# Z1HaoC/YOLO-Dual

Measured on AMD Instinct MI355X. Metric: images/sec at 640x640 bs=16/GPU, higher is better.
Workload: dtype bf16; 1 GPU; YOLOv5-backbone (C3+SPPF) + UNet-lite SegmentHead, fwd+bwd+SGD/EMA step, 640x640, bs=16/GPU, CE+0.5*Dice, 12 classes (BASELINE configs[1]); global_batch=16, parallelism=dp1

## Files before the change

### yolo_dual_amd/csrc/igemm.hip

```cpp
#include "common.h"
#include <type_traits>
#include <stdlib.h>

#ifndef YDL_PF
#define YDL_PF 1
#endif
#define ROWB 144
#define GROWB 128
#define MAXTAPS 64

struct IgemmArgs {
    const void* A;
    const void* B;
    void* C;
    float* stats;
    int N, Hi, Wi, lda;
    int Kc;
    int Ho, Wo, ldc;
    int Cout;
    int Cst;
    int Hg, Wg;
    int in_mul, out_mul, out_h0, out_w0;
    int ntaps, Ttot;
    int accumulate;
// ... 1504 lines not shown
        browoff[i] = co < p.Cout ? (unsigned)co * p.ldb_bytes + (unsigned)((qs ^ ((row >> 1) & 7)) << 4) : 0xF0000000u;
    }
    const int spt = p.Kc >> 6;
    const int nsteps = 9 * spt;
    u32x4 rsA, rsB;
    {
        const unsigned long long pa = (unsigned long long)p.A, pb = (unsigned long long)p.B;
        rsA = u32x4{(unsigned)pa, (unsigned)(pa >> 32) & 0xffffu, p.bytesA, 0x00020000u};
        rsB = u32x4{(unsigned)pb, (unsigned)(pb >> 32) & 0xffffu, p.bytesB, 0x00020000u};
    }
    const unsigned lds0 = (unsigned)(size_t)(__attribute__((address_space(3))) unsigned char*)smem;
    const unsigned wave_lds = lds0 + (unsigned)wave * (8 * GROWB);
    auto issue_patch = [&](int cb) {
        const unsigned base = wave_lds + (unsigned)(ONEP ? 0 : (cb & 1)) * PBYTES;
        const unsigned kb = (unsigned)cb << 7;
#pragma unroll
        for (int i = 0; i < PP; ++i) {
            if (RPP * i + wave * 8 < HS_PROWS)
                lds_dma16(rsA, base + i * RPP * GROWB, poff[i] == 0xFFFFFFFFu ? 0xFFFFFFFFu : poff[i] + kb);
        }
    };
    auto issue_w = [&](int stg, int cbw, int woff) {
        const unsigned add = cbw < spt ? (unsigned)woff + ((unsigned)cbw << 7) : 0xF0000000u;
        const unsigned base = wave_lds + (unsigned)NPB * PBYTES + (unsigned)stg * RBYTES;
#pragma unroll
        for (int i = 0; i < BR; ++i) lds_dma16(rsB, base + i * RPP * GROWB, browoff[i] + add);
    };
    f32x4 acc[CT][PT];
#pragma unroll
    for (int c = 0; c < CT; ++c)
#pragma unroll
        for (int j = 0; j < PT; ++j) acc[c][j] = f32x4{0.f, 0.f, 0.f, 0.f};
    const int lrow = lane & 15, lgrp = lane >> 4;
    const int sw_w = (lrow >> 1) & 7;
    const unsigned char* const fa = ring + (wc * BNW + lrow) * GROWB;
    issue_patch(0);
    issue_w(0, 0, sTw[0]);
    int cb = 0, tap = 0;
    int dcur = sTd[0], wnx = sTw[1];
    for (int g = 0; g < nsteps; ++g) {
        asm volatile("s_waitcnt lgkmcnt(0)" ::: "memory");
        wait_vm_barrier<0>();
        const int t1 = tap == 8 ? 0 : tap + 1, c1 = tap == 8 ? cb + 1 : cb;
        const int t2 = t1 == 8 ? 0 : t1 + 1;
        const int dnx = sTd[t1], wnn = sTw[t2];
        issue_w((g + 1) & 1, c1, wnx);
        if constexpr (ONEP) {
            if (tap == 0 && cb > 0) {
                issue_patch(cb);
                wait_vm_barrier<0>();
            }
        } else {
            if (tap == 0 && cb + 1 < spt) issue_patch(cb + 1);
        }
        const unsigned char* const wst = fa + (g & 1) * RBYTES;
        const unsigned char* const pst = smem + (ONEP ? 0 : (cb & 1)) * PBYTES;
        int prow[PT];
#pragma unroll
        for (int j = 0; j < PT; ++j) prow[j] = (wp * PT + j + 1) * H_PW + (lrow + 1) + dcur;
#pragma unroll
        for (int half = 0; half < 2; ++half) {
            uint4 af[CT], bfr[PT];
            const int kq = lgrp + 4 * half;
#pragma unroll
            for (int c = 0; c < CT; ++c) af[c] = *(const uint4*)(wst + c * 16 * GROWB + ((kq ^ sw_w) << 4));
#pragma unroll
            for (int j = 0; j < PT; ++j) bfr[j] = *(const uint4*)(pst + prow[j] * GROWB + ((kq ^ ((prow[j] >> 1) & 7)) << 4));
#pragma unroll
            for (int c = 0; c < CT; ++c)
#pragma unroll
                for (int j = 0; j < PT; ++j) Mma<T>::run(af[c], bfr[j], acc[c][j]);
        }
        dcur = dnx; wnx = wnn; tap = t1; cb = c1;
    }
    asm volatile("s_waitcnt lgkmcnt(0)" ::: "memory");
    wait_vm_barrier<0>();
    igemm2_epilogue<BM, BN, NW, WP>(p, acc, smem, 0, n0, mtile, BM, 16, 8, n * p.Ho + h0, w0);
}

__device__ __forceinline__ void buf_store16_asm(const u32x4& v, unsigned off, const u32x4& rsrc) {
    asm volatile("buffer_store_dwordx4 %0, %1, %2, 0 offen\n\ts_nop 1" ::"v"(v), "v"(off), "s"(rsrc) : "memory");
}
#define WR_PW 34
typedef __attribute__((ext_vector_type(16))) float f32x16_t;
template <int CO, bool STATS, int NW>
__global__ __launch_bounds__(NW * 64, 2) void igemm2w_kernel(const IgemmArgs p, int nblocks) {
    using T = bf16_t;
    constexpr int CG = CO / 32, PG = NW / CG, RW = 2, R = PG * RW;
    constexpr int NT = NW * 64, PR = NW * 8;
    constexpr int PROWS = (R + 2) * WR_PW;
    constexpr int PASSES = (PROWS + PR - 1) / PR;
    constexpr int PBYTES = PASSES * PR * GROWB;
    constexpr int BPX = R * 32;
    constexpr int NCH = CO / 8;
    constexpr int ORB = CO * 2;
    static_assert(BPX * NCH == 4 * NT && NT % NCH == 0, "four 16-byte store slots per thread, a fixed channel chunk per thread");
    extern __shared__ __attribute__((aligned(16))) unsigned char smem[];
    unsigned char* const stage = smem + 2 * PBYTES;
    float* const sred = (float*)smem;
    const int t = threadIdx.x, lane = t & 63;
    const int wave = __builtin_amdgcn_readfirstlane(t >> 6);
    const int cg = wave % CG, pg = wave / CG;
    const int ln = lane & 31, lh = lane >> 5;
    const int blocks_w = p.Wo >> 5, blocks_img = (p.Ho / R) * blocks_w;
    u32x4 rsA, rsC;
    {
        const unsigned long long pa = (unsigned long long)p.A, pc = (unsigned long long)p.C;
        rsA = u32x4{(unsigned)pa, (unsigned)(pa >> 32) & 0xffffu, p.bytesA, 0x00020000u};
        rsC = u32x4{(unsigned)pc, (unsigned)(pc >> 32) & 0xffffu, p.bytesC, 0x00020000u};
    }
    const unsigned lds0 = (unsigned)(size_t)(__attribute__((address_space(3))) unsigned char*)smem;
    const unsigned wave_lds = lds0 + (unsigned)wave * 1024u;
    const int rq = t >> 3, qs = t & 7;
    int pprc[PASSES];
#pragma unroll
    for (int i = 0; i < PASSES; ++i) {
        const int rho = i * PR + rq;
        pprc[i] = rho < PROWS ? ((rho / WR_PW) << 8) | (rho - (rho / WR_PW) * WR_PW) : (4000000 << 8);
    }
    auto block_origin = [&](int b, int& n, int& h0, int& w0) {
        n = b / blocks_img;
        const int rem = b - n * blocks_img;
        h0 = (rem / blocks_w) * R;
        w0 = (rem % blocks_w) << 5;
    };
    auto issue_patch = [&](int b, int buf) {
        int n, h0, w0;
        block_origin(b, n, h0, w0);
        const bool live = b < nblocks;
#pragma unroll
        for (int i = 0; i < PASSES; ++i) {
            const int rho = i * PR + rq;
            const int h = h0 - 1 + (pprc[i] >> 8), w = w0 - 1 + (pprc[i] & 255);
            const bool ok = live && (unsigned)h < (unsigned)p.Hi && (unsigned)w < (unsigned)p.Wi;
            const unsigned off = (unsigned)(((n * p.Hi + h) * p.Wi + w) * p.lda) * 2u + (unsigned)((qs ^ ((rho >> 1) & 7)) << 4);
            lds_dma16(rsA, wave_lds + (unsigned)buf * PBYTES + (unsigned)(i * PR * GROWB), ok ? off : 0xFFFFFFFFu);
        }
    };
    const int per = (nblocks + (int)gridDim.x - 1) / (int)gridDim.x;
    const int b0 = blockIdx.x * per, b1 = min(nblocks, b0 + per);
    issue_patch(b0, 0);
    uint4 wreg[9][4];
    {
        const __amdgpu_buffer_rsrc_t rsB = __builtin_amdgcn_make_buffer_rsrc((void*)p.B, 0, p.bytesB, 0x00020000);
        const int co = cg * 32 + ln;
#pragma unroll
        for (int tp = 0; tp < 9; ++tp)
#pragma unroll
            for (int ks = 0; ks < 4; ++ks) {
                const unsigned off = co < p.Cout ? (unsigned)co * p.ldb_bytes + (unsigned)(((int)p.wt[tp] * p.Kc + ks * 16 + lh * 8) * 2) : 0xFFFFFFFFu;
                const u32x4 v = __builtin_amdgcn_raw_buffer_load_b128(rsB, off, 0, 0);
                wreg[tp][ks] = make_uint4(v.x, v.y, v.z, v.w);
            }
    }
    int tapd[9];
#pragma unroll
    for (int tp = 0; tp < 9; ++tp) tapd[tp] = (int)p.dh[tp] * WR_PW + (int)p.dw[tp];
    float s1[STATS ? 8 : 1], s2[STATS ? 8 : 1];
#pragma unroll
    for (int e = 0; e < (STATS ? 8 : 1); ++e) { s1[e] = 0.f; s2[e] = 0.f; }
    const bool want_stats = STATS && p.stats != nullptr;
    int ridx_base = (pg * RW + 1) * WR_PW + ln + 1;
    asm volatile("s_waitcnt vmcnt(0)\n\ts_barrier" ::: "memory");
    int buf = 0;
    for (int b = b0; b < b1; ++b, buf ^= 1) {
        issue_patch(b + 1 < b1 ? b + 1 : nblocks, buf ^ 1);
        const unsigned char* const pst = smem + buf * PBYTES;
        f32x16_t acc[RW];
#pragma unroll
        for (int rb = 0; rb < RW; ++rb)
#pragma unroll
            for (int e = 0; e < 16; ++e) acc[rb][e] = 0.f;
        asm volatile("" : "+v"(ridx_base));
        uint4 fq[2][4];
        auto rd = [&](int tp, int rb, uint4 (&f)[4]) {
            const int ridx = ridx_base + rb * WR_PW + tapd[tp];
            const unsigned char* const rowp = pst + ridx * GROWB;
            const int sw = (ridx >> 1) & 7;
#pragma unroll
            for (int ks = 0; ks < 4; ++ks) f[ks] = *(const uint4*)(rowp + (((2 * ks + lh) ^ sw) << 4));
        };
        rd(0, 0, fq[0]);
#pragma unroll
        for (int step = 0; step < 9 * RW; ++step) {
            const int tp = step / RW, rb = step % RW;
            if (step + 1 < 9 * RW) rd((step + 1) / RW, (step + 1) % RW, fq[(step + 1) & 1]);
#pragma unroll
            for (int ks = 0; ks < 4; ++ks)
                acc[rb] = __builtin_amdgcn_mfma_f32_32x32x16_bf16(__builtin_bit_cast(bf16x8, wreg[tp][ks]),
                                                                  __builtin_bit_cast(bf16x8, fq[step & 1][ks]), acc[rb], 0, 0, 0);
            __builtin_amdgcn_sched_barrier(0);
        }
#pragma unroll
        for (int rb = 0; rb < RW; ++rb) {
            const int px = (pg * RW + rb) * 32 + ln;
#pragma unroll
            for (int g = 0; g < 4; ++g) {
                uint2 u;
                u.x = (uint32_t)f2bf(acc[rb][4 * g + 0]) | ((uint32_t)f2bf(acc[rb][4 * g + 1]) << 16);
                u.y = (uint32_t)f2bf(acc[rb][4 * g + 2]) | ((uint32_t)f2bf(acc[rb][4 * g + 3]) << 16);
                const int chq = cg * 4 + g;
                *(uint2*)(stage + px * ORB + ((chq ^ (px & (NCH - 1))) << 4) + (lh << 3)) = u;
            }
        }
        asm volatile("s_waitcnt lgkmcnt(0)\n\ts_barrier" ::: "memory");
        {
            int n, h0, w0;
            block_origin(b, n, h0, w0);
#pragma unroll
            for (int j = 0; j < 4; ++j) {
                const int idx = t + NT * j;
                const int px = idx / NCH, ch = idx % NCH;
                const uint4 v = *(const uint4*)(stage + px * ORB + ((ch ^ (px & (NCH - 1))) << 4));
                if constexpr (STATS) {
                    if (want_stats) {
                        float f[8];
                        unpack16<T>(v, f);
#pragma unroll
                        for (int e = 0; e < 8; ++e) { s1[e] += f[e]; s2[e] = fmaf(f[e], f[e], s2[e]); }
                    }
                }
                const unsigned m = (unsigned)((n * p.Ho + h0 + (px >> 5)) * p.Wo + w0 + (px & 31));
                const unsigned off = ch * 8 < p.Cst ? (m * (unsigned)p.ldc + (unsigned)(ch * 8)) * 2u : 0xFFFFFFFFu;
                asm volatile("s_waitcnt lgkmcnt(0)" ::: "memory");
                buf_store16_asm(u32x4{v.x, v.y, v.z, v.w}, off, rsC);
            }
        }
        asm volatile("s_waitcnt vmcnt(4)\n\ts_barrier" ::: "memory");
    }
    if constexpr (!STATS) {
        asm volatile("s_waitcnt vmcnt(0)" ::: "memory");
        return;
    }
    if (want_stats) {
#pragma unroll
        for (int e = 0; e < (STATS ? 8 : 1); ++e)
#pragma unroll
            for (int o = NCH; o < 64; o <<= 1) { s1[e] += __shfl_xor(s1[e], o, 64); s2[e] += __shfl_xor(s2[e], o, 64); }
        asm volatile("s_waitcnt vmcnt(0) lgkmcnt(0)\n\ts_barrier" ::: "memory");
        if (lane < NCH) {
#pragma unroll
            for (int e = 0; e < (STATS ? 8 : 1); ++e) {
                sred[(wave * CO + lane * 8 + e) * 2] = s1[e];
                sred[(wave * CO + lane * 8 + e) * 2 + 1] = s2[e];
            }
        }
        __syncthreads();
        if (t < CO && t < p.Cout) {
            float a = 0.f, b2 = 0.f;
#pragma unroll
            for (int w = 0; w < NW; ++w) { a += sred[(w * CO + t) * 2]; b2 += sred[(w * CO + t) * 2 + 1]; }
            float* dst = p.stats + (size_t)(blockIdx.x & (YDL_BN_REPLICAS - 1)) * 2 * p.stats_ld;
            atomicAdd(dst + t, a);
            atomicAdd(dst + p.stats_ld + t, b2);
        }
    } else {
        asm volatile("s_waitcnt vmcnt(0)" ::: "memory");
    }
}

static int g_wreg = 1;
static bool wreg_ok(const IgemmArgs& a) {
    static const int env = getenv("YDL_WREG") ? atoi(getenv("YDL_WREG")) : 1;
    if (!env || !g_wreg || a.br.nseg > 0 || a.accumulate) return false;
    if (a.ncls > 1 || a.ntaps != 9 || a.Ttot != 9 || a.in_mul != 1 || a.out_mul != 1 || a.out_h0 != 0 || a.out_w0 != 0) return false;
    if (a.Hi != a.Ho || a.Wi != a.Wo || a.Hg != a.Ho || a.Wg != a.Wo || a.Kc != 64) return false;
    if (a.Cst != 64 && a.Cst != 128) return false;
    if ((a.Wo & 31) || a.Ho % (a.Cst == 128 ? 4 : 8)) return false;
    if (a.stats != nullptr && !a.stats_atomic) return false;
    if ((long long)a.M < 4ll * 128 * ydl_device_cus()) return false;
    bool seen[9] = {false, false, false, false, false, false, false, false, false};
    for (int t = 0; t < 9; ++t) {
        const int dh = a.dh[t], dw = a.dw[t];
        if (dh < -1 || dh > 1 || dw < -1 || dw > 1 || seen[(dh + 1) * 3 + dw + 1]) return false;
        seen[(dh + 1) * 3 + dw + 1] = true;
    }
    return true;
}
template <int CO, int NW>
static int launch_igemm2w_cfg(IgemmArgs a, hipStream_t st, int fam) {
    constexpr int R = (NW / (CO / 32)) * 2, PR = NW * 8;
    const int nblocks = a.N * (a.Ho / R) * (a.Wo >> 5);
    constexpr int PASSES = ((R + 2) * WR_PW + PR - 1) / PR;
    const size_t smem = 2 * (size_t)PASSES * PR * GROWB + (size_t)R * 32 * CO * 2;
    YDL_SET_MAX_LDS((igemm2w_kernel<CO, true, NW>), smem);
    YDL_SET_MAX_LDS((igemm2w_kernel<CO, false, NW>), smem);
    const unsigned long long bc = ((unsigned long long)(a.N * a.Ho * a.Wo - 1) * a.ldc + a.Cst) * 2ull;
    YDL_CHECK(bc < 0xFFFFFFF0ull, "output larger than 4 GiB");
    a.bytesC = (unsigned)bc;
    static const std::string nm = std::string("igemm2w_kernel<") + std::to_string(CO) + (NW == 8 ? ">" : ",nw4>");
    ydl_note_kernel(fam, nm.c_str());
    const int ctas = std::min(ydl_device_cus() * (NW == 8 ? 1 : 2), nblocks);
    if (a.stats != nullptr) igemm2w_kernel<CO, true, NW><<<ctas, NW * 64, smem, st>>>(a, nblocks);
    else igemm2w_kernel<CO, false, NW><<<ctas, NW * 64, smem, st>>>(a, nblocks);
    YDL_LAUNCH_CHECK();
    return 0;
}
static int launch_igemm2w(const IgemmArgs& a, hipStream_t st, int fam) {
    static const int nw = getenv("YDL_WREG_NW") ? atoi(getenv("YDL_WREG_NW")) : 4;
    if (nw == 4) return a.Cst == 128 ? launch_igemm2w_cfg<128, 4>(a, st, fam) : launch_igemm2w_cfg<64, 4>(a, st, fam);
    return a.Cst == 128 ? launch_igemm2w_cfg<128, 8>(a, st, fam) : launch_igemm2w_cfg<64, 8>(a, st, fam);
}

#define S2_PW 17
#define S2_PROWS 192
__device__ constexpr int kS2Kh[9] = {1, 1, 2, 2, 1, 2, 0, 0, 0};
__device__ constexpr int kS2Kw[9] = {1, 2, 1, 2, 0, 0, 1, 2, 0};
template <int NW, int WP, int S, bool ACC>
__global__ __launch_bounds__(NW * 64, NW / 2) void igemm2s_kernel(const IgemmArgs p) {
    using T = bf16_t;
    constexpr int ES = 2;
    constexpr int BM = 128, BN = 64;
    constexpr int RPP = NW * 8;
    constexpr int BR = BN / RPP;
    constexpr int PP = (S2_PROWS + RPP - 1) / RPP;
    constexpr int WN = NW / WP;
    constexpr int BNW = BN / WN;
    constexpr int CT = BNW / 16;
    constexpr int PT = BM / (16 * WP);
    constexpr int PBYTES = S2_PROWS * GROWB;
    constexpr int RBYTES = BN * GROWB;
    static_assert(BN % RPP == 0 && BR == 1 && S2_PROWS % RPP == 0 && (S == 2 || S == 3), "one weight DMA per thread and step, whole patch passes");
    static_assert(2 * PBYTES + S * RBYTES >= BM * BN * 2, "epilogue scratch");
    extern __shared__ __attribute__((aligned(16))) unsigned char smem[];
    unsigned char* const ring = smem + 2 * PBYTES;
    const int t = threadIdx.x;
    const int lane = t & 63;
    const int wave = __builtin_amdgcn_readfirstlane(t >> 6);
    const int wc = wave % WN, wp = wave / WN;
    const int tile = xcd_remap(blockIdx.x, gridDim.x);
    const int mtile = tile / p.grid_n, ntile = tile - mtile * p.grid_n;
    const int tiles_w = p.Wi >> 4, tiles_hw = (p.Hi >> 3) * tiles_w;
    const int n = mtile / tiles_hw;
    const int rem = mtile - n * tiles_hw;
    const int i0 = (rem / tiles_w) << 3, j0 = (rem % tiles_w) << 4;
    const int n0 = ntile * BN;
    const int r = t >> 3, qs = t & 7;
    const unsigned browoff = (n0 + r) < p.Cout ? (unsigned)(n0 + r) * p.ldb_bytes + (unsigned)((qs ^ ((r >> 1) & 7)) << 4) : 0xF0000000u;
    const int spt = p.Kc >> 6;
    u32x4 rsA, rsB;
    {
        const unsigned long long pa = (unsigned long long)p.A, pb = (unsigned long long)p.B;
        rsA = u32x4{(unsigned)pa, (unsigned)(pa >> 32) & 0xffffu, p.bytesA, 0x00020000u};
        rsB = u32x4{(unsigned)pb, (unsigned)(pb >> 32) & 0xffffu, p.bytesB, 0x00020000u};
    }
    const unsigned lds0 = (unsigned)(size_t)(__attribute__((address_space(3))) unsigned char*)smem;
    const unsigned wave_lds = lds0 + (unsigned)wave * (8 * GROWB);
    auto issue_patch = [&](int cb) {
        const unsigned base = wave_lds + (unsigned)(cb & 1) * PBYTES;
        const unsigned kb = (unsigned)cb << 7;
        const bool live = cb < spt;
#pragma unroll
        for (int i = 0; i < PP; ++i) {
            const int rho = r + RPP * i;
            const int pr = rho / S2_PW, pc = rho - pr * S2_PW;
            const int h = i0 + pr, w = j0 + pc;
            const bool ok = live && rho < 9 * S2_PW && h < p.Hi && w < p.Wi;
            const unsigned off = (unsigned)(((n * p.Hi + h) * p.Wi + w) * p.lda) * (unsigned)ES + (unsigned)((qs ^ ((rho >> 1) & 7)) << 4) + kb;
            lds_dma16(rsA, base + i * RPP * GROWB, ok ? off : 0xFFFFFFFFu);
        }
    };
    auto issue_w = [&](int stg, int cb, int slice) {
        const unsigned add = cb < spt ? (unsigned)slice * (unsigned)p.Kc * ES + ((unsigned)cb << 7) : 0xF0000000u;
        lds_dma16(rsB, wave_lds + 2u * PBYTES + (unsigned)stg * RBYTES, browoff + add);
    };
    f32x4 acc[4][CT][PT];
#pragma unroll
    for (int q = 0; q < 4; ++q)
#pragma unroll
        for (int c = 0; c < CT; ++c)
#pragma unroll
            for (int j = 0; j < PT; ++j) acc[q][c][j] = f32x4{0.f, 0.f, 0.f, 0.f};
    const int lrow = lane & 15, lgrp = lane >> 4;
    const int sw_w = (lrow >> 1) & 7;
    const unsigned char* const fa = ring + (wc * BNW + lrow) * GROWB;
    uint4 bq[2][PT];
    auto step = [&](auto ic, int cb) {
        constexpr int I = decltype(ic)::value;
        constexpr int kh = kS2Kh[I], kw = kS2Kw[I];
        constexpr int dh = kh == 0 ? 1 : 0, dw = kw == 0 ? 1 : 0;
        constexpr int cls = (kh != 1 ? 2 : 0) + (kw != 1 ? 1 : 0);
        constexpr bool group_start = I == 0 || I == 4 || I == 6 || I == 8;
        constexpr int I1 = (I + 8) % 9, I2 = (I + 7) % 9;
        constexpr int NY = S == 2 ? 0 : 1 + (I1 == 0 ? PP : 0) + (I2 == 0 ? PP : 0);
// ... 830 lines not shown
        case 14: return launch_igemm2<128, 128, 8, 4, 2, false, 1>(a, st, fam);
        case 15: return launch_igemm2<256, 128, 8, 4, 3, false, 1>(a, st, fam);
        case 16: return launch_igemm2<256, 128, 8, 4, 2, false, 1>(a, st, fam);
        case 17: return launch_igemm2<128, 128, 8, 4, 2, false, 2>(a, st, fam);
        case 18: return launch_igemm2<256, 128, 8, 4, 3, false, 2>(a, st, fam);
        case 19: return launch_igemm2<256, 128, 8, 4, 3, false, 3>(a, st, fam);
        case 24: return launch_igemm2l<256, 128, 8, 4, 3, 4>(a, st, fam);
        case 25: return launch_igemm2l<128, 128, 8, 4, 3, 4>(a, st, fam);
        case 29: return launch_igemm2l<128, 128, 4, 2, 2, 4>(a, st, fam);
        case 23: return launch_igemm2<256, 128, 4, 2, 3>(a, st, fam);
    }
    ydl_set_error("internal: unknown ring kernel id");
    return 1;
}

static TileCfg pick_cfg(int M, int Cst, int nchunks = 0, bool bf16 = false, int Kc = 0, int taps = 0, bool one_class = true, bool loaders_ok = true) {
    TileCfg c;
    c.ring = 0;
    static const int ring64 = getenv("YDL_RING64") ? atoi(getenv("YDL_RING64")) : 13;
    if (bf16 && g_ring_enabled && Cst >= (ring64 ? 64 : 128) && Cst % 8 == 0 && nchunks >= 16 && Kc > 0 && Kc % 64 == 0 && taps <= 29) {
        static const int forced = getenv("YDL_RING") ? atoi(getenv("YDL_RING")) : -1;
        const long b128 = (long)((M + 127) / 128) * ((Cst + 127) / 128);
        int id = b128 < 256 ? 9 : 7;
        static const int big = getenv("YDL_RING256") ? atoi(getenv("YDL_RING256")) : 1;
        const long b256 = (long)((M + 255) / 256) * ((Cst + 127) / 128);
        if (big && one_class && Cst >= 128 && b256 >= 180 && b256 <= 512 && nchunks >= 96) id = 15;
        if (ring_loaders() && loaders_ok) {
            if (id == 15 && nchunks >= 128) id = 24;
            if (id == 9 && b128 >= 64) id = 25;
            if (id == 7 && b128 < 1280) id = 29;
        }
        if (Cst < 128) id = ring64;
        if (forced >= 0) id = forced;
        if (id > 0) { c.ring = id; c.BM = kRingBM[id]; c.BN = kRingBN[id]; return c; }
    }
    c.BN = Cst <= 16 ? 16 : (Cst <= 64 ? 64 : 128);
    c.BM = 128;
    long blocks = (long)((M + 127) / 128) * ((Cst + c.BN - 1) / c.BN);
    if (blocks < 512 && c.BN == 128) {
        long b1 = (long)((M + 127) / 128) * ((Cst + 63) / 64);
        if (b1 >= 512) { c.BN = 64; return c; }
    }
    if (blocks < 512 && c.BN != 16) c.BM = 64;
    if (c.BM == 64 && c.BN == 128) {
        long b2 = (long)((M + 63) / 64) * ((Cst + 127) / 128);
        if (b2 < 512) c.BN = 64;
    }
    return c;
}

template <typename T>
static int dispatch_igemm(const IgemmArgs& a, hipStream_t st, int fam, FwdRows* rows_out = nullptr, int force_bm = 0, int* path_out = nullptr) {
    if constexpr (sizeof(T) == 2) {
        if (fam == 0 && !force_bm && args_stem(a)) {
            const StemPlan sp = stem_plan(a.M, a.Wo);
            if (sp.ok && path_out) { *path_out = 3; return 0; }
            if (sp.ok && rows_out) { *rows_out = FwdRows{sp.grid_m, sp.block_m}; return 0; }
            if (sp.ok) {
                StemArgs q{};
                q.X = (const bf16_t*)a.A; q.W = (const bf16_t*)a.B; q.Y = (bf16_t*)a.C; q.stats = a.stats;
                q.H = a.Hi; q.Wd = a.Wi; q.ldc = a.ldc; q.M = a.M; q.block_m = sp.block_m; q.stats_ld = a.stats_ld;
                q.stats_atomic = a.stats_atomic; q.bytesX = a.bytesA;
                ydl_note_kernel(fam, "stem_kernel<bf16,16,64>");
                stem_kernel<<<sp.grid_m, 256, 0, st>>>(q);
                YDL_LAUNCH_CHECK();
                return 0;
            }
        }
    }
    {
        const PwPlan pl = pw_plan(a.M, a.Kc, a.Cout, a.Cst, (int)sizeof(T), args_pointwise(a));
        if (pl.ok && !force_bm && path_out) { *path_out = 1; return 0; }
        if (pl.ok && !force_bm && rows_out) { *rows_out = FwdRows{pl.grid_m, pl.block_m}; return 0; }
        if (pl.ok && !force_bm) {
            YDL_CHECK(a.br.nseg == 0, "fused BatchNorm reduce: this geometry runs on the point-wise kernel (query ydl_conv_dgrad_bnred_supported)");
            PwArgs q{};
            q.X = a.A; q.W = a.B; q.Y = a.C; q.stats = a.stats;
            q.M = a.M; q.lda = a.lda; q.ldc = a.ldc; q.Cout = a.Cout; q.WN = pl.WN; q.accumulate = a.accumulate;
            q.block_m = pl.block_m; q.stats_ld = a.stats_ld; q.stats_atomic = a.stats_atomic; q.bytesX = a.bytesA; q.ldw_bytes = a.ldb_bytes;
            return launch_pw<T>(q, pl, st, fam);
        }
    }
    if constexpr (sizeof(T) == 2) {
        if (!force_bm && !path_out && wreg_ok(a)) {
            YDL_CHECK(rows_out == nullptr, "internal: the weights-in-registers kernel writes no statistics partial rows");
            return launch_igemm2w(a, st, fam);
        }
    }
    int nch = a.ntaps * (a.Kc / (16 / (int)sizeof(T)));
    if (a.ncls > 1) {
        nch = 1 << 30;
        for (int i = 0; i < a.ncls; ++i) nch = min(nch, a.cls_ntaps[i] * (a.Kc / (16 / (int)sizeof(T))));
    }
    TileCfg c = pick_cfg(a.M, a.Cst, nch, sizeof(T) == 2, a.Kc, a.Ttot, a.ncls <= 1, a.br.nseg == 0 && path_out == nullptr);
    if constexpr (sizeof(T) == 2) {
        if (c.ring && !force_bm) {
            if (path_out) { *path_out = ring_has_bnred(c.ring) ? 2 : 4; return 0; }
            return launch_ring(c.ring, a, st, fam, rows_out);
        }
    }
    if (path_out) { *path_out = 0; return 0; }
    YDL_CHECK(a.br.nseg == 0, "fused BatchNorm reduce: this geometry runs on the register-staged kernel (query ydl_conv_dgrad_bnred_supported)");
    if (c.ring) c = pick_cfg(a.M, a.Cst);
    if (force_bm) c.BM = force_bm;
    static const int env_bm = getenv("YDL_FORCE_BM") ? atoi(getenv("YDL_FORCE_BM")) : 0;
    static const int env_bn = getenv("YDL_FORCE_BN") ? atoi(getenv("YDL_FORCE_BN")) : 0;
    if (env_bm && a.stats == nullptr) c.BM = env_bm;
    if (env_bn && c.BN != 16 && a.Cst >= env_bn) c.BN = env_bn;
    if (rows_out) { *rows_out = FwdRows{(a.M + c.BM - 1) / c.BM, c.BM}; return 0; }
    static const int nw8 = getenv("YDL_NW8") ? atoi(getenv("YDL_NW8")) : 1;
    if (c.BM == 128 && c.BN == 128) {
        if (nw8 == 2) return launch_igemm<T, 128, 128, 4, 2>(a, st, fam);
        return nw8 ? launch_igemm<T, 128, 128, 8>(a, st, fam) : launch_igemm<T, 128, 128, 4>(a, st, fam);
    }
    if (c.BM == 128 && c.BN == 64) return launch_igemm<T, 128, 64>(a, st, fam);
    if (c.BM == 128 && c.BN == 16) return launch_igemm<T, 128, 16>(a, st, fam);
    if (c.BM == 64 && c.BN == 128) return nw8 ? launch_igemm<T, 64, 128, 8>(a, st, fam) : launch_igemm<T, 64, 128, 4>(a, st, fam);
    if (c.BM == 64 && c.BN == 64) return launch_igemm<T, 64, 64>(a, st, fam);
    return launch_igemm<T, 64, 16>(a, st, fam);
}

static int set_extents(IgemmArgs& a, int dtype) {
    const unsigned long long es = (unsigned long long)esize(dtype);
    unsigned long long ba = (unsigned long long)a.N * a.Hi * a.Wi * a.lda * es;
    if (a.ldb_bytes == 0) a.ldb_bytes = (unsigned)((unsigned long long)a.Ttot * a.Kc * es);
    unsigned long long bb = (unsigned long long)(a.Cout - 1) * a.ldb_bytes + (unsigned long long)a.Ttot * a.Kc * es;
    YDL_CHECK(ba < 0xFFFFFFF0ull && bb < 0xFFFFFFF0ull, "tensor larger than 4 GiB: not addressable by the 32-bit buffer loads");
    a.bytesA = (unsigned)ba;
    a.bytesB = (unsigned)bb;
    return 0;
}

static int check_geom(const ydl_conv_geom* g, int dtype) {
    YDL_CHECK(g != nullptr, "null geometry");
    YDL_CHECK(dtype == YDL_F32 || dtype == YDL_BF16, "bad dtype");
    YDL_CHECK(g->N > 0 && g->Hi > 0 && g->Wi > 0 && g->Cin > 0 && g->Cout > 0, "non-positive dims");
    YDL_CHECK(g->k >= 1 && g->k * g->k <= MAXTAPS && g->s >= 1 && g->p >= 0, "unsupported kernel/stride/pad");
    YDL_CHECK(g->Ho == (g->Hi + 2 * g->p - g->k) / g->s + 1 && g->Wo == (g->Wi + 2 * g->p - g->k) / g->s + 1,
              "output size does not match (H+2p-k)/s+1");
    int es = esize(dtype);
    YDL_CHECK(g->ldx >= round_up(g->Cin, 8) && g->ldy >= g->Cout, "pixel stride smaller than channel count");
    YDL_CHECK((g->ldx * es) % 16 == 0 && (g->ldy * es) % 16 == 0, "pixel strides must be 16-byte multiples");
    YDL_CHECK((int64_t)g->N * g->Hi * g->Wi < (1ll << 31) && (int64_t)g->N * g->Ho * g->Wo < (1ll << 31), "too many pixels");
    YDL_CHECK(g->ldw == 0 || (g->ldw >= g->k * g->k * round_up(g->Cin, 8) && (g->ldw * es) % 16 == 0),
              "ldw must be 0 (dense) or a 16-byte-multiple row stride >= k*k*round_up(Cin, 8)");
    return 0;
}

static int fwd_args(const ydl_conv_geom* g, int dtype, const void* x, const void* w, void* y, float* stats_ws, int stats_atomic,
                    int accumulate, IgemmArgs& a) {
    if (int e = check_geom(g, dtype)) return e;
    a = IgemmArgs{};
    a.A = x; a.B = w; a.C = y; a.stats = stats_ws;
    a.N = g->N; a.Hi = g->Hi; a.Wi = g->Wi; a.lda = g->ldx;
    a.Kc = round_up(g->Cin, 8);
    a.Ho = g->Ho; a.Wo = g->Wo; a.ldc = g->ldy; a.Cout = g->Cout;
    a.Cst = round_up(g->Cout, 8) <= g->ldy ? round_up(g->Cout, 8) : g->Cout;
    a.Hg = g->Ho; a.Wg = g->Wo; a.in_mul = g->s; a.out_mul = 1; a.out_h0 = 0; a.out_w0 = 0;
    a.ntaps = g->k * g->k; a.Ttot = a.ntaps; a.accumulate = accumulate ? 1 : 0;
    a.M = g->N * g->Ho * g->Wo;
    a.stats_ld = round_up(g->Cout, 8);
    a.stats_atomic = stats_atomic;
    a.ldb_bytes = (unsigned)(g->ldw * esize(dtype));
    for (int r = 0; r < g->k; ++r)
        for (int s = 0; s < g->k; ++s) {
            int tpi = r * g->k + s;
            a.dh[tpi] = (signed char)(r - g->p); a.dw[tpi] = (signed char)(s - g->p); a.wt[tpi] = (unsigned char)tpi;
        }
    return set_extents(a, dtype);
// ... 1323 lines not shown
        const int stages = (M + 63) / 64;
        if (mid) {
            static const long slots = getenv("YDL_WG2_MIDSLOTS") ? atol(getenv("YDL_WG2_MIDSLOTS")) : 512;
            int splits = (int)(slots / tiles);
            const int per = (stages + splits - 1) / splits;
            pl.chunk = per * 64;
            pl.splits = (M + pl.chunk - 1) / pl.chunk;
            return pl;
        }
        static const long forced = getenv("YDL_WG2_CTAS") ? atol(getenv("YDL_WG2_CTAS")) : 0;
        long target2 = forced;
        if (!target2) {
            const double bytes_in = ((double)g->N * g->Hi * g->Wi * g->Cin + (double)M * g->Cout) * 2.0;
            const double flops = 2.0 * M * g->Cout * ntaps * Kc;
            const double d0 = bytes_in / 4.5e12 > flops / 450e12 ? bytes_in / 4.5e12 : flops / 450e12;
            const double share = Kc <= 16 ? 0.3 : 0.2;
            const double t = share * d0 * 1.3e12 / (128.0 * TCO * 4.0);
            target2 = (long)(t / 256.0 + 0.5) * 256;
            if (target2 < 256) target2 = 256;
            if (target2 > 2048) target2 = 2048;
        }
        int splits = (int)((target2 + tiles - 1) / tiles);
        if (splits > stages / 4) splits = stages / 4;
        if (splits < 1) splits = 1;
        if (splits > 1024) splits = 1024;
        const int per = (stages + splits - 1) / splits;
        pl.chunk = per * 64;
        pl.splits = (M + pl.chunk - 1) / pl.chunk;
        return pl;
    }
    pl.kind = dtype == YDL_F32 ? 0 : (g_wgrad_tr ? 1 : 2);
    const int TE = dtype == YDL_F32 ? 32 : 64;
    pl.jtiles = (ntaps * Kc + TE - 1) / TE;
    pl.ctiles = (g->Cout + TE - 1) / TE;
    const long tiles = (long)pl.jtiles * pl.ctiles;
    const int stages = (M + WG_BKP - 1) / WG_BKP;
    static const long forced_ctas = getenv("YDL_WG_CTAS") ? atol(getenv("YDL_WG_CTAS")) : 0;
    const long target_ctas = forced_ctas ? forced_ctas : (ntaps == 1 ? 1024 : 2048);
    static const long atomic_budget = getenv("YDL_WG_ATOMIC_MB") ? atol(getenv("YDL_WG_ATOMIC_MB")) * (1l << 20) : (1l << 40);
    int splits = (int)((target_ctas + tiles - 1) / tiles);
    const long dw_bytes = (long)g->Cout * ntaps * Kc * 4;
    if ((long)splits * dw_bytes > atomic_budget) splits = (int)(atomic_budget / dw_bytes);
    if (splits > stages / 4) splits = stages / 4;
    if (splits < 1) splits = 1;
    if (splits > 1024) splits = 1024;
    const int per = (stages + splits - 1) / splits;
    pl.chunk = per * WG_BKP;
    pl.splits = (M + pl.chunk - 1) / pl.chunk;
    return pl;
}

__global__ __launch_bounds__(256) void wgrad_reduce_kernel(const float* __restrict__ slab, float* __restrict__ dW, int splits,
                                                           int Cout, int wrow, int ldw) {
    const size_t n = (size_t)Cout * wrow;
    for (size_t i = (size_t)blockIdx.x * 256 + threadIdx.x; i < n; i += (size_t)gridDim.x * 256) {
        float s = 0.f;
        for (int z = 0; z < splits; ++z) s += slab[(size_t)z * n + i];
        const size_t co = i / wrow, j = i - co * wrow;
        dW[co * ldw + j] += s;
    }
}

extern int g_resize_int, g_resize_rows;
void ydl_dcn_debug_set(int key, int val);
void ydl_deform_debug_set(int key, int val);
extern "C" void ydl_debug_set(int key, int val) {
    ydl_dcn_debug_set(key, val);
    ydl_deform_debug_set(key, val);
    if (key == 0) g_wgrad_tr = val;
    if (key == 1) g_pw_enabled = val;
    if (key == 2) g_dgrad_merge = val;
    if (key == 3) g_ring_enabled = val;
    if (key == 4) g_wgrad_dma = val;
    if (key == 5) g_stem_enabled = val;
    if (key == 6) g_ring_persist = val;
    if (key == 8) g_halo = val;
    if (key == 9) g_s2fused = val;
    if (key == 10) g_resize_int = val;
    if (key == 11) g_resize_rows = val;
    if (key == 12) g_stemw = val;
    if (key == 14) g_pw_acc_ts = val;
    if (key == 15) g_pwbw = val;
    if (key == 17) g_wreg = val;
    if (key == 18) g_wg3_loaders = val;
    if (key == 19) g_ring_loaders = val;
}

extern "C" int64_t ydl_conv_wgrad_ws_bytes(const ydl_conv_geom* g, int dtype) {
    if (g == nullptr || g->Cin <= 0 || g->Cout <= 0 || g->k < 1) return 0;
    const WgradPlan pl = wgrad_plan(g, dtype);
    return (int64_t)pl.splits * g->Cout * (int64_t)(g->k * g->k * round_up(g->Cin, 8)) * (int64_t)sizeof(float);
}

static int conv_wgrad_impl(const ydl_conv_geom* g, int dtype, const void* x, const void* dy, float* dw, float* slab, void* stream) {
    if (int e = check_geom(g, dtype)) return e;
    YDL_CHECK(aligned16(x) && aligned16(dy) && aligned16(dw), "pointers must be 16-byte aligned");
    const int V = dtype == YDL_F32 ? 4 : 8;
    YDL_CHECK(g->ldy >= round_up(g->Cout, V), "dy pixel stride must cover Cout rounded up to a 16-byte chunk");
    const WgradPlan pl = wgrad_plan(g, dtype);
    const int Kc = round_up(g->Cin, 8), ntaps = g->k * g->k;
    const int M = g->N * g->Ho * g->Wo;
    const unsigned long long es = (unsigned long long)esize(dtype);
    const unsigned long long bx = (unsigned long long)g->N * g->Hi * g->Wi * g->ldx * es, by = (unsigned long long)M * g->ldy * es;
    YDL_CHECK(bx < 0xFFFFFFF0ull && by < 0xFFFFFFF0ull && (unsigned long long)M * ((unsigned long long)g->Ho * g->Wo) < (1ull << 40),
              "tensor too large for the 32-bit wgrad addressing");
    YDL_CHECK(g->Ho < (1 << 21) && g->Wo < (1 << 21), "map side of 2^21 or more: not supported by the weight-gradient kernels (24-bit row / column arithmetic)");
    const unsigned long long magicW = ((1ull << 40) + g->Wo - 1) / g->Wo;
    const unsigned long long magicHW = ((1ull << 40) + (unsigned long long)g->Ho * g->Wo - 1) / ((unsigned long long)g->Ho * g->Wo);
    const int ldw = g->ldw ? g->ldw : ntaps * Kc;
    hipStream_t st = (hipStream_t)stream;
    dim3 grid(pl.jtiles * pl.ctiles * pl.splits);
    if (slab == nullptr && stemw_ok(g, dtype)) return launch_stemw(g, x, dy, dw, ldw, (unsigned)bx, (unsigned)by, st);
    if (pl.kind >= 3) {
        Wgrad2Args a{};
        a.X = (const bf16_t*)x; a.dY = (const bf16_t*)dy; a.dW = dw;
        a.N = g->N; a.Hi = g->Hi; a.Wi = g->Wi; a.ldx = g->ldx; a.Kc = Kc;
        a.Ho = g->Ho; a.Wo = g->Wo; a.ldy = g->ldy; a.Cout = g->Cout;
        a.k = g->k; a.s = g->s; a.p = g->p; a.ntaps = ntaps;
        a.ldw = ldw; a.M = M; a.chunk = pl.chunk;
        a.bytesX = (unsigned)bx; a.bytesY = (unsigned)by; a.magicW = magicW; a.magicHW = magicHW;
        a.njt = pl.jtiles; a.nct = pl.ctiles; a.slab = slab;
        static const int w3dbg = getenv("YDL_WG3_DBG") ? atoi(getenv("YDL_WG3_DBG")) : 0;
        a.dbg = w3dbg;
        static const int dma_env = getenv("YDL_WG3") ? atoi(getenv("YDL_WG3")) : 1;
        if (g_wgrad_dma && dma_env) {
            static const int cfg = getenv("YDL_WG3_CFG") ? atoi(getenv("YDL_WG3_CFG")) : 1;
            ydl_note_kernel(2, pl.kind == 4 ? "wgrad3_kernel<128>" : "wgrad3_kernel<64>");
            int e = 0;
            const int loaders = wg3_loaders();
            if (loaders) ydl_note_kernel(2, pl.kind == 4 ? "wgrad3s_kernel<128>" : "wgrad3s_kernel<64>");
            if (loaders == 1 || loaders == 2 || loaders == 4) {
                if (pl.kind == 4) e = loaders == 1 ? launch_wgrad3s<128, 32, 4, 1>(a, grid, st) : (loaders == 2 ? launch_wgrad3s<128, 32, 4, 2>(a, grid, st) : launch_wgrad3s<128, 32, 4, 4>(a, grid, st));
                else e = loaders == 1 ? launch_wgrad3s<64, 32, 4, 1>(a, grid, st) : (loaders == 2 ? launch_wgrad3s<64, 32, 4, 2>(a, grid, st) : launch_wgrad3s<64, 32, 4, 4>(a, grid, st));
            } else
            if (pl.kind == 4) e = cfg == 0 ? launch_wgrad3<128, 64, 2>(a, grid, st) : (cfg == 2 ? launch_wgrad3<128, 64, 3>(a, grid, st) : launch_wgrad3<128, 32, 4>(a, grid, st));
            else e = cfg == 0 ? launch_wgrad3<64, 64, 2>(a, grid, st) : (cfg == 2 ? launch_wgrad3<64, 64, 3>(a, grid, st) : launch_wgrad3<64, 32, 4>(a, grid, st));
            if (e) return e;
        } else {
            const size_t smem = 4 * 64 * W2_ROWB;
            YDL_SET_MAX_LDS((wgrad2_kernel<128>), smem);
            YDL_SET_MAX_LDS((wgrad2_kernel<64>), smem);
            ydl_note_kernel(2, pl.kind == 4 ? "wgrad2_kernel<128>" : "wgrad2_kernel<64>");
            if (pl.kind == 4) wgrad2_kernel<128><<<grid, 256, smem, st>>>(a);
            else wgrad2_kernel<64><<<grid, 256, smem, st>>>(a);
            YDL_LAUNCH_CHECK();
        }
    } else {
        WgradArgs a{};
        a.X = x; a.dY = dy; a.dW = dw;
        a.N = g->N; a.Hi = g->Hi; a.Wi = g->Wi; a.ldx = g->ldx; a.Kc = Kc;
        a.Ho = g->Ho; a.Wo = g->Wo; a.ldy = g->ldy; a.Cout = g->Cout;
        a.k = g->k; a.s = g->s; a.p = g->p; a.ntaps = ntaps;
        a.ldw = ldw; a.M = M; a.chunk = pl.chunk;
        a.bytesX = (unsigned)bx; a.bytesY = (unsigned)by; a.magicW = magicW; a.magicHW = magicHW;
        a.njt = pl.jtiles; a.nct = pl.ctiles; a.slab = slab;
        if (pl.kind == 0) { ydl_note_kernel(2, "wgrad_kernel<f32>"); wgrad_kernel<float, false><<<grid, 256, 0, st>>>(a); }
        else if (pl.kind == 1) { ydl_note_kernel(2, "wgrad_kernel<bf16,tr>"); wgrad_kernel<bf16_t, true><<<grid, 256, 0, st>>>(a); }
        else { ydl_note_kernel(2, "wgrad_kernel<bf16,scalar>"); wgrad_kernel<bf16_t, false><<<grid, 256, 0, st>>>(a); }
        YDL_LAUNCH_CHECK();
    }
    if (slab) {
        const int wrow = ntaps * Kc;
        const size_t n = (size_t)g->Cout * wrow;
        int blocks = (int)((n + 255) / 256);
        if (blocks > 2048) blocks = 2048;
        wgrad_reduce_kernel<<<blocks, 256, 0, st>>>(slab, dw, pl.splits, g->Cout, wrow, ldw);
// ... 15 lines not shown
```

Baseline: 2601 images/sec.

## Extend weights-in-registers 3x3 conv kernel to stride-2 with deinterleaved patch

Adds a stride-2 variant of the weights-in-registers implicit-GEMM conv kernel for 64-in/128-out channel layers. The input patch is loaded into LDS with even and odd columns split apart so each tap reads contiguous rows, and the geometry is factored into a template struct. The aim is to move stride-2 downsampling convs off the generic ring or register-staged path onto the faster register-resident weight kernel. Each block now covers a single output row per wave group, which means fewer pixels per block and a different store count.

```diff
diff --git a/yolo_dual_amd/csrc/igemm.hip b/yolo_dual_amd/csrc/igemm.hip
--- a/yolo_dual_amd/csrc/igemm.hip
+++ b/yolo_dual_amd/csrc/igemm.hip
@@ -1610,19 +1610,32 @@
     asm volatile("buffer_store_dwordx4 %0, %1, %2, 0 offen\n\ts_nop 1" ::"v"(v), "v"(off), "s"(rsrc) : "memory");
 }
 #define WR_PW 34
+#define WS_PW 65
 typedef __attribute__((ext_vector_type(16))) float f32x16_t;
-template <int CO, bool STATS, int NW>
+template <int CO, int NW, int S>
+struct WregGeom {
+    static constexpr int CG = CO / 32, PG = NW / CG;
+    static constexpr int RW = S == 1 ? 2 : 1, R = PG * RW;
+    static constexpr int PW = S == 1 ? WR_PW : WS_PW;
+    static constexpr int PROWS = (S == 1 ? R + 2 : 2 * R + 1) * PW;
+    static constexpr int PR = NW * 8;
+    static constexpr int PASSES = (PROWS + PR - 1) / PR;
+    static constexpr int PBYTES = PASSES * PR * GROWB;
+    static constexpr int BPX = R * 32;
+    static constexpr size_t SMEM = 2 * (size_t)PBYTES + (size_t)BPX * CO * 2;
+};
+template <int CO, bool STATS, int NW, int S>
 __global__ __launch_bounds__(NW * 64, 2) void igemm2w_kernel(const IgemmArgs p, int nblocks) {
     using T = bf16_t;
-    constexpr int CG = CO / 32, PG = NW / CG, RW = 2, R = PG * RW;
-    constexpr int NT = NW * 64, PR = NW * 8;
-    constexpr int PROWS = (R + 2) * WR_PW;
-    constexpr int PASSES = (PROWS + PR - 1) / PR;
-    constexpr int PBYTES = PASSES * PR * GROWB;
-    constexpr int BPX = R * 32;
+    using G = WregGeom<CO, NW, S>;
+    constexpr int CG = G::CG, PG = G::PG, RW = G::RW, R = G::R, PW = G::PW;
+    constexpr int NT = NW * 64, PR = G::PR;
+    constexpr int PROWS = G::PROWS, PASSES = G::PASSES, PBYTES = G::PBYTES;
+    constexpr int BPX = G::BPX;
     constexpr int NCH = CO / 8;
     constexpr int ORB = CO * 2;
-    static_assert(BPX * NCH == 4 * NT && NT % NCH == 0, "four 16-byte store slots per thread, a fixed channel chunk per thread");
+    constexpr int NST = BPX * NCH / NT;
+    static_assert(BPX * NCH == NST * NT && (NST == 4 || NST == 2) && NT % NCH == 0, "whole store slots per thread, a fixed channel chunk per thread");
     extern __shared__ __attribute__((aligned(16))) unsigned char smem[];
     unsigned char* const stage = smem + 2 * PBYTES;
     float* const sred = (float*)smem;
@@ -1643,8 +1656,9 @@
     int pprc[PASSES];
 #pragma unroll
     for (int i = 0; i < PASSES; ++i) {
-        const int rho = i * PR + rq;
-        pprc[i] = rho < PROWS ? ((rho / WR_PW) << 8) | (rho - (rho / WR_PW) * WR_PW) : (4000000 << 8);
+        const int rho = i * PR + rq, pr = rho / PW, pc = rho - pr * PW;
+        const int col = S == 1 ? pc : (pc < 33 ? 2 * pc : 2 * (pc - 33) + 1);
+        pprc[i] = rho < PROWS ? (pr << 8) | col : (4000000 << 8);
     }
     auto block_origin = [&](int b, int& n, int& h0, int& w0) {
         n = b / blocks_img;
@@ -1659,7 +1673,7 @@
 #pragma unroll
         for (int i = 0; i < PASSES; ++i) {
             const int rho = i * PR + rq;
-            const int h = h0 - 1 + (pprc[i] >> 8), w = w0 - 1 + (pprc[i] & 255);
+            const int h = S * h0 - 1 + (pprc[i] >> 8), w = S * w0 - 1 + (pprc[i] & 255);
             const bool ok = live && (unsigned)h < (unsigned)p.Hi && (unsigned)w < (unsigned)p.Wi;
             const unsigned off = (unsigned)(((n * p.Hi + h) * p.Wi + w) * p.lda) * 2u + (unsigned)((qs ^ ((rho >> 1) & 7)) << 4);
             lds_dma16(rsA, wave_lds + (unsigned)buf * PBYTES + (unsigned)(i * PR * GROWB), ok ? off : 0xFFFFFFFFu);
@@ -1683,12 +1697,14 @@
     }
     int tapd[9];
 #pragma unroll
-    for (int tp = 0; tp < 9; ++tp) tapd[tp] = (int)p.dh[tp] * WR_PW + (int)p.dw[tp];
+    for (int tp = 0; tp < 9; ++tp)
+        tapd[tp] = S == 1 ? (int)p.dh[tp] * WR_PW + (int)p.dw[tp]
+                          : ((int)p.dh[tp] + 1) * WS_PW + (p.dw[tp] == 0 ? 33 : ((int)p.dw[tp] + 1) >> 1);
     float s1[STATS ? 8 : 1], s2[STATS ? 8 : 1];
 #pragma unroll
     for (int e = 0; e < (STATS ? 8 : 1); ++e) { s1[e] = 0.f; s2[e] = 0.f; }
     const bool want_stats = STATS && p.stats != nullptr;
-    int ridx_base = (pg * RW + 1) * WR_PW + ln + 1;
+    int ridx_base = S == 1 ? (pg * RW + 1) * WR_PW + ln + 1 : pg * RW * 2 * WS_PW + ln;
     asm volatile("s_waitcnt vmcnt(0)\n\ts_barrier" ::: "memory");
     int buf = 0;
     for (int b = b0; b < b1; ++b, buf ^= 1) {
@@ -1702,7 +1718,7 @@
         asm volatile("" : "+v"(ridx_base));
         uint4 fq[2][4];
         auto rd = [&](int tp, int rb, uint4 (&f)[4]) {
-            const int ridx = ridx_base + rb * WR_PW + tapd[tp];
+            const int ridx = ridx_base + rb * S * PW + tapd[tp];
             const unsigned char* const rowp = pst + ridx * GROWB;
             const int sw = (ridx >> 1) & 7;
 #pragma unroll
@@ -1736,7 +1752,7 @@
             int n, h0, w0;
             block_origin(b, n, h0, w0);
 #pragma unroll
-            for (int j = 0; j < 4; ++j) {
+            for (int j = 0; j < NST; ++j) {
                 const int idx = t + NT * j;
                 const int px = idx / NCH, ch = idx % NCH;
                 const uint4 v = *(const uint4*)(stage + px * ORB + ((ch ^ (px & (NCH - 1))) << 4));
@@ -1754,7 +1770,7 @@
                 buf_store16_asm(u32x4{v.x, v.y, v.z, v.w}, off, rsC);
             }
         }
-        asm volatile("s_waitcnt vmcnt(4)\n\ts_barrier" ::: "memory");
+        wait_vm_barrier<NST>();
     }
     if constexpr (!STATS) {
         asm volatile("s_waitcnt vmcnt(0)" ::: "memory");
@@ -1788,46 +1804,54 @@
 }
 
 static int g_wreg = 1;
-static bool wreg_ok(const IgemmArgs& a) {
+static int g_wreg_s2 = 1;
+static int wreg_ok(const IgemmArgs& a) {
     static const int env = getenv("YDL_WREG") ? atoi(getenv("YDL_WREG")) : 1;
-    if (!env || !g_wreg || a.br.nseg > 0 || a.accumulate) return false;
-    if (a.ncls > 1 || a.ntaps != 9 || a.Ttot != 9 || a.in_mul != 1 || a.out_mul != 1 || a.out_h0 != 0 || a.out_w0 != 0) return false;
-    if (a.Hi != a.Ho || a.Wi != a.Wo || a.Hg != a.Ho || a.Wg != a.Wo || a.Kc != 64) return false;
-    if (a.Cst != 64 && a.Cst != 128) return false;
-    if ((a.Wo & 31) || a.Ho % (a.Cst == 128 ? 4 : 8)) return false;
-    if (a.stats != nullptr && !a.stats_atomic) return false;
-    if ((long long)a.M < 4ll * 128 * ydl_device_cus()) return false;
+    static const int env_s2 = getenv("YDL_WREG_S2") ? atoi(getenv("YDL_WREG_S2")) : 1;
+    if (a.br.nseg > 0 || a.accumulate) return 0;
+    if (a.ncls > 1 || a.ntaps != 9 || a.Ttot != 9 || a.out_mul != 1 || a.out_h0 != 0 || a.out_w0 != 0) return 0;
+    if (a.Hg != a.Ho || a.Wg != a.Wo || a.Kc != 64) return 0;
+    int s = 0;
+    if (a.in_mul == 1 && env && g_wreg && a.Hi == a.Ho && a.Wi == a.Wo && (a.Cst == 64 || a.Cst == 128)) {
+        if (a.Ho % (a.Cst == 128 ? 4 : 8)) return 0;
+        s = 1;
+    }
+    if (a.in_mul == 2 && env_s2 && g_wreg_s2 && a.Cst == 128) s = 2;
+    if (s == 0 || (a.Wo & 31)) return 0;
+    if (a.stats != nullptr && !a.stats_atomic) return 0;
+    if ((long long)a.M < 4ll * 128 * ydl_device_cus()) return 0;
     bool seen[9] = {false, false, false, false, false, false, false, false, false};
     for (int t = 0; t < 9; ++t) {
         const int dh = a.dh[t], dw = a.dw[t];
-        if (dh < -1 || dh > 1 || dw < -1 || dw > 1 || seen[(dh + 1) * 3 + dw + 1]) return false;
+        if (dh < -1 || dh > 1 || dw < -1 || dw > 1 || seen[(dh + 1) * 3 + dw + 1]) return 0;
         seen[(dh + 1) * 3 + dw + 1] = true;
     }
-    return true;
-}
-template <int CO, int NW>
+    return s;
+}
+template <int CO, int NW, int S>
 static int launch_igemm2w_cfg(IgemmArgs a, hipStream_t st, int fam) {
-    constexpr int R = (NW / (CO / 32)) * 2, PR = NW * 8;
-    const int nblocks = a.N * (a.Ho / R) * (a.Wo >> 5);
-    constexpr int PASSES = ((R + 2) * WR_PW + PR - 1) / PR;
-    const size_t smem = 2 * (size_t)PASSES * PR * GROWB + (size_t)R * 32 * CO * 2;
-    YDL_SET_MAX_LDS((igemm2w_kernel<CO, true, NW>), smem);
-    YDL_SET_MAX_LDS((igemm2w_kernel<CO, false, NW>), smem);
+    using G = WregGeom<CO, NW, S>;
+    static_assert(NW * CO * 2 * sizeof(float) <= 2 * (size_t)G::PBYTES, "statistics scratch in the patch buffers");
+    const int nblocks = a.N * (a.Ho / G::R) * (a.Wo >> 5);
+    const size_t smem = G::SMEM;
+    YDL_SET_MAX_LDS((igemm2w_kernel<CO, true, NW, S>), smem);
+    YDL_SET_MAX_LDS((igemm2w_kernel<CO, false, NW, S>), smem);
     const unsigned long long bc = ((unsigned long long)(a.N * a.Ho * a.Wo - 1) * a.ldc + a.Cst) * 2ull;
     YDL_CHECK(bc < 0xFFFFFFF0ull, "output larger than 4 GiB");
     a.bytesC = (unsigned)bc;
-    static const std::string nm = std::string("igemm2w_kernel<") + std::to_string(CO) + (NW == 8 ? ">" : ",nw4>");
+    static const std::string nm = std::string("igemm2w_kernel<") + std::to_string(CO) + (NW == 8 ? "" : ",nw4") + (S == 2 ? ",s2>" : ">");
     ydl_note_kernel(fam, nm.c_str());
     const int ctas = std::min(ydl_device_cus() * (NW == 8 ? 1 : 2), nblocks);
-    if (a.stats != nullptr) igemm2w_kernel<CO, true, NW><<<ctas, NW * 64, smem, st>>>(a, nblocks);
-    else igemm2w_kernel<CO, false, NW><<<ctas, NW * 64, smem, st>>>(a, nblocks);
+    if (a.stats != nullptr) igemm2w_kernel<CO, true, NW, S><<<ctas, NW * 64, smem, st>>>(a, nblocks);
+    else igemm2w_kernel<CO, false, NW, S><<<ctas, NW * 64, smem, st>>>(a, nblocks);
     YDL_LAUNCH_CHECK();
     return 0;
 }
-static int launch_igemm2w(const IgemmArgs& a, hipStream_t st, int fam) {
+static int launch_igemm2w(const IgemmArgs& a, int stride, hipStream_t st, int fam) {
+    if (stride == 2) return launch_igemm2w_cfg<128, 4, 2>(a, st, fam);
     static const int nw = getenv("YDL_WREG_NW") ? atoi(getenv("YDL_WREG_NW")) : 4;
-    if (nw == 4) return a.Cst == 128 ? launch_igemm2w_cfg<128, 4>(a, st, fam) : launch_igemm2w_cfg<64, 4>(a, st, fam);
-    return a.Cst == 128 ? launch_igemm2w_cfg<128, 8>(a, st, fam) : launch_igemm2w_cfg<64, 8>(a, st, fam);
+    if (nw == 4) return a.Cst == 128 ? launch_igemm2w_cfg<128, 4, 1>(a, st, fam) : launch_igemm2w_cfg<64, 4, 1>(a, st, fam);
+    return a.Cst == 128 ? launch_igemm2w_cfg<128, 8, 1>(a, st, fam) : launch_igemm2w_cfg<64, 8, 1>(a, st, fam);
 }
 
 #define S2_PW 17
@@ -2824,9 +2848,10 @@
         }
     }
     if constexpr (sizeof(T) == 2) {
-        if (!force_bm && !path_out && wreg_ok(a)) {
+        const int wst = (!force_bm && !path_out) ? wreg_ok(a) : 0;
+        if (wst) {
             YDL_CHECK(rows_out == nullptr, "internal: the weights-in-registers kernel writes no statistics partial rows");
-            return launch_igemm2w(a, st, fam);
+            return launch_igemm2w(a, wst, st, fam);
         }
     }
     int nch = a.ntaps * (a.Kc / (16 / (int)sizeof(T)));
@@ -4316,6 +4341,7 @@
     if (key == 14) g_pw_acc_ts = val;
     if (key == 15) g_pwbw = val;
     if (key == 17) g_wreg = val;
+    if (key == 21) g_wreg_s2 = val;
     if (key == 18) g_wg3_loaders = val;
     if (key == 19) g_ring_loaders = val;
 }
```

After: 2601 images/sec, median of 6. Within noise of the previous version (+0.0%).
